# aniketntnu/WordDiffusion

Hardware: AMD Instinct MI355X
Metric: denoised 64x256 word images/sec (1000-step DDPM), whole job (higher is better)
Workload: dtype bf16x3; 1 GPU; BASELINE configs[1]: batch 64 per GPU of 64x256 crops = [64,4,8,32] latents, 1000-step DDPM (999 executed steps), base unet.py UNetModel (320 ch, mult (1,1), 4 heads, 339 writers), random-init synthetic weights; variant=base, batch_per_gpu=64, noise_steps=1000, executed_steps_per_image=999, precision=split-bf16 MFMA x3, fp32 accumulate (<=1e-4 of the fp32 reference), output_finite=True

## Files before the change

include/wdiff_hip.h:

```cpp
#ifndef WDIFF_HIP_H
#define WDIFF_HIP_H

#include <stdint.h>

#ifdef __cplusplus
extern "C" {
#endif

#define WD_OK 0
#define WD_EINVAL (-1)
#define WD_ELAUNCH (-2)
#define WD_ESTATE (-3)

#define WD_ACT_NONE 0
#define WD_ACT_SILU 1
#define WD_ACT_GEGLU 2

typedef uint16_t wd_bf16;

#define WD_MAX_KSPLIT 64

typedef struct wd_src {
    const wd_bf16* hi;
    const wd_bf16* lo;
// ... 173 lines not shown
                   const wd_bf16* mq_pl, const wd_bf16* mot_pl, void* stream);

int wd_emb_combine(const float* time, const float* label, const int64_t* y, int num_classes, int T, int B, int ted,
                   wd_bf16* out_hi, wd_bf16* out_lo, int out_ld, void* stream);
int wd_select_rows(const float* table, const int32_t* t_dev, int batch, int64_t row_floats, int chunk, float* out,
                   void* stream);

int wd_emb_combine_mix(const float* time, const float* label, const int32_t* pairs, const float* mix, int num_classes, int T, int B,
                       int ted, wd_bf16* out_hi, wd_bf16* out_lo, int out_ld, void* stream);
int wd_label_mix(const float* label, const int32_t* pairs, const float* mix, int num_classes, int B, int ted, float* out,
                 void* stream);

int wd_xattn_pair(const float* x, int ld, int batch, int hw, int c, float eps, int heads, int L, const float* gamma_a,
                  const float* beta_a, const wd_bf16* mq_pl_a, const wd_bf16* mot_pl_a, const float* bias_a, const float* gamma_b,
                  const float* beta_b, const wd_bf16* mq_pl_b, const wd_bf16* mot_pl_b, const float* bias_b, float* out, int out_ld,
                  const float* gamma2, const float* beta2, float eps2, wd_bf16* n_hi, wd_bf16* n_lo, int n_ld, void* stream);

int wd_embed_tokens(const void* ids, int ids_are_i64, int rows, int seq_len, const float* table, int vocab, int c,
                    const float* pe, wd_bf16* out_hi, wd_bf16* out_lo, int out_ld, void* stream);

int wd_im2col3x3(const float* x, int batch, int cin, int h, int w, wd_bf16* out_hi, wd_bf16* out_lo, int kpad,
                 void* stream);

int wd_nchw_to_tokens(const float* x, int batch, int c, int hw, float* out, int ld, void* stream);
int wd_tokens_to_nchw(const float* x, int ld, int batch, int c, int hw, float* out, void* stream);

int wd_ddpm_step(float* x, const float* eps, int batch, int n_per_sample, const float* ca, const float* cb,
                 const float* cs, const int32_t* t_dev, const float* noise, uint64_t seed, uint64_t sample_offset,
                 void* stream);

int wd_ddpm_step_cfg(float* x, const float* first, const float* second, float scale, float* eps_out, int batch, int n_per_sample,
                     const float* ca, const float* cb, const float* cs, const int32_t* t_dev, const float* noise, uint64_t seed,
                     uint64_t sample_offset, void* stream);

int wd_advance_timestep(int32_t* t_dev, int delta, int64_t* t64, int batch, void* stream);

int wd_ddim_step(float* x, const float* eps, const float* second, float scale, float* eps_out, int batch, int n_per_sample,
                 const float* c1, const float* c2, const float* c3, const float* c4, const float* c5, const int32_t* k_dev,
                 const int32_t* t_dev, const float* noise, uint64_t seed, uint64_t sample_offset, void* stream);

int wd_next_timestep(int32_t* k_dev, const int32_t* tau, int S, int32_t* t_dev, int64_t* t64, int batch, void* stream);

int wd_randn(float* out, int batch, int n_per_sample, uint64_t seed, uint64_t sample_offset, uint32_t stream_id,
             void* stream);

#define WD_VAE_MAX_LATENT 8
// ... 142 lines not shown
```

worddiffusion_amd/_native.py:

```python
from __future__ import annotations

import ctypes as C
import os
import re

_HERE = os.path.dirname(os.path.abspath(__file__))
LIB_PATH = os.environ.get("WDIFF_LIB") or os.path.join(_HERE, "libwdiff_hip.so")
HEADER_PATH = os.path.join(os.path.dirname(_HERE), "include", "wdiff_hip.h")

WD_OK, WD_EINVAL, WD_ELAUNCH, WD_ESTATE = 0, -1, -2, -3
ACT_NONE, ACT_SILU, ACT_GEGLU = 0, 1, 2
VAE_MAX_LATENT, STREAM_VAE_POSTERIOR = 8, 3
NCLASS = 13
CLASS_NAMES = ("gemm", "gn_stats", "gn_apply", "layernorm", "attention", "other", "gemm_other_tiles", "gemm_splitk_reduce",
               "gemm_two_per_cu", "gemm_weights_to_registers", "feed_forward_fused", "weight_gradient", "gemm_small_maps_whole_k")

_vp = C.c_void_p
_i = C.c_int
_f = C.c_float
_u64 = C.c_uint64


class WdSrc(C.Structure):
    _fields_ = [("hi", _vp), ("lo", _vp), ("gather", _vp), ("ld", C.c_int32), ("c", C.c_int32),
# ... 56 lines not shown
    "wd_gemm_pack_w": (_i, [_vp, _vp, _i, _i, _vp, _vp, _vp]),
    "wd_ff_fused": (_i, [C.POINTER(WdFfArgs), _vp]),
    "wd_ff_supported": (_i, [_i, _i]),
    "wd_ff_args_bytes": (_i, []),
    "wd_gemm_args_bytes": (_i, []),
    "wd_gemm_experimental": (_i, []),
    "wd_gn_nchunk": (_i, [_i]),
    "wd_gn_stats": (_i, [_vp, _i, _i, _i, _i, _i, _vp, _vp]),
    "wd_gn_fold_chunks": (_i, [_vp, _i, _i, _i, _vp, _vp]),
    "wd_gn_conv3x3_few_supported": (_i, [_i, _i, _i]),
    "wd_gn_conv3x3_few": (_i, [_vp, _i, _i, _i, _i, _i, _i, _vp, _i, _i, _vp, _vp, _f, _i, _vp, _vp, _i, _vp, _vp]),
    "wd_gn_apply": (_i, [_vp, _i, _i, _i, _i, _i, _vp, _i, _i, _vp, _vp, _f, _i, _vp, _vp, _i, _i, _vp, _vp, _vp]),
    "wd_gn_apply2": (_i, [_vp, _i, _i, _vp, _i, _i, _i, _vp, _i, _i, _vp, _i, _i, _i, _i, _i, _i, _vp, _vp, _f, _i, _vp, _vp, _i, _vp,
                          _vp, _vp, _vp]),
    "wd_layernorm": (_i, [_vp, _i, _i, _i, _vp, _vp, _f, _vp, _vp, _i, _vp]),
    "wd_split": (_i, [_vp, _i, _i, _i, _i, _vp, _vp, _i, _vp]),
    "wd_attention": (_i, [_vp, _i, _vp, _i, _vp, _i, _i, _i, _i, _i, _i, _f, _vp, _vp, _vp, _i, _i, _i, _vp]),
    "wd_attention_packed_elems": (C.c_int64, [_i, _i, _i, _i]),
    "wd_attention_pack_kv": (_i, [_vp, _i, _vp, _i, _i, _i, _i, _i, _vp, _vp]),
    "wd_attention_packed": (_i, [_vp, _i, _vp, _i, _i, _i, _i, _i, _f, _vp, _vp, _vp, _i, _i, _i, _vp]),
    "wd_timestep_embedding": (_i, [_vp, _i, _vp, _i, _vp, _vp, _i, _vp]),
    "wd_embed_tokens": (_i, [_vp, _i, _i, _i, _vp, _i, _i, _vp, _vp, _vp, _i, _vp]),
    "wd_im2col3x3": (_i, [_vp, _i, _i, _i, _i, _vp, _vp, _i, _vp]),
    "wd_nchw_to_tokens": (_i, [_vp, _i, _i, _i, _vp, _i, _vp]),
    "wd_tokens_to_nchw": (_i, [_vp, _i, _i, _i, _i, _vp, _vp]),
    "wd_ddpm_step": (_i, [_vp, _vp, _i, _i, _vp, _vp, _vp, _vp, _vp, _u64, _u64, _vp]),
    "wd_advance_timestep": (_i, [_vp, _i, _vp, _i, _vp]),
    "wd_randn": (_i, [_vp, _i, _i, _u64, _u64, C.c_uint32, _vp]),
    "wd_vae_posterior": (_i, [_vp, _i, _vp, _vp, _i, _i, _i, _vp, _vp, _vp, _f, _vp, _u64, _u64, _vp]),
    "wd_posterior_sample": (_i, [_vp, _vp, _i, _i, _vp, _f, _vp, _u64, _u64, _vp]),
    "wd_noise_images": (_i, [_vp, _vp, _vp, _vp, _vp, _i, _i, _vp, _vp]),
    "wd_copy2d": (_i, [_vp, C.c_int64, _vp, C.c_int64, C.c_int64, C.c_int64, _vp]),
    "wd_ema_update": (_i, [_vp, _vp, C.c_int64, C.c_double, _vp]),
    "wd_adamw_table_entry_bytes": (_i, []),
    "wd_adamw_chunk": (_i, []),
    "wd_adamw_multi": (_i, [_vp, _i, C.c_int64, C.c_double, C.c_double, C.c_double, C.c_double, C.c_double, C.c_int64, _i,
                           C.c_double, _vp]),
    "wd_mse_loss": (_i, [_vp, _vp, C.c_int64, _vp, _vp, _vp, _i, _vp]),
    "wd_transpose_planes": (_i, [_vp, _vp, _i, _i, _i, _vp, _i, _i, _i, _i, _i, _i, _vp, _vp, _vp]),
    "wd_repack_entry_bytes": (_i, []),
    "wd_repack_tile": (_i, []),
    "wd_repack_vchunk": (_i, []),
    "wd_repack_multi": (_i, [_vp, _i, C.c_int64, _vp]),
    "wd_attention_bwd_scratch_floats": (C.c_int64, [_i, _i, _i, _i]),
    "wd_attention_bwd": (_i, [_vp, _i, _vp, _i, _vp, _i, _vp, _i, _i, _i, _i, _i, _i, _f, _vp, _i, _vp, _i, _vp, _i, _vp, C.c_int64, _vp]),
    "wd_xattn_supported": (_i, [_i, _i, _i]),
# ... 95 lines not shown
```

worddiffusion_amd/build.py:

```python
from __future__ import annotations

import hashlib
import json
import os
import subprocess
import sys
from concurrent.futures import ThreadPoolExecutor

HERE = os.path.dirname(os.path.abspath(__file__))
CSRC = os.path.join(HERE, "csrc")
LIB = os.path.join(HERE, "libwdiff_hip.so")
SOURCES = ["wd_gemm.hip", "wd_gemmw.hip", "wd_gemmq.hip", "wd_ff.hip", "wd_dw.hip", "wd_norm.hip", "wd_attn.hip", "wd_xattn.hip", "wd_misc.hip", "wd_train.hip", "wd_bwd.hip", "wd_pack.hip", "wd_runtime.hip"]
HEADERS = [os.path.join(CSRC, "wd_common.h"), os.path.join(CSRC, "wd_gemm_epi.h"), os.path.join(CSRC, "wd_gemm_priv.h"), os.path.join(os.path.dirname(HERE), "include", "wdiff_hip.h")]
FLAGS = ["-O3", "--offload-arch=gfx950", "-fPIC", "-std=c++17", "-fno-gpu-rdc"]
FILE_FLAGS = {"wd_attn.hip": ["-mllvm", "-amdgpu-mfma-vgpr-form=1"]}
if os.environ.get("WDIFF_EXPERIMENTAL", "0") != "0":
    FLAGS.append("-DWDIFF_EXPERIMENTAL")
if os.environ.get("WDIFF_STAMPS", "0") != "0":
    FLAGS += ["-DWD_DW_STAMPS", "-DWD_GEMMW_STAMPS", "-DWD_Q_STAMPS"]


def _hipcc() -> str:
    for cand in (os.environ.get("HIPCC"), "/opt/rocm/bin/hipcc", "hipcc"):
        if cand and (os.path.isabs(cand) and os.path.exists(cand) or not os.path.isabs(cand)):
            return cand
    return "hipcc"


def _digest(paths) -> str:
    h = hashlib.sha256()
    for p in paths:
        with open(p, "rb") as f:
            h.update(hashlib.sha256(f.read()).digest())
    h.update(" ".join(FLAGS + FILE_FLAGS.get(os.path.basename(paths[0]), [])).encode())
    return h.hexdigest()
# ... 55 lines not shown
```

worddiffusion_amd/csrc/wd_norm.hip:

```cpp
#include "wd_common.h"

namespace {

constexpr int GN_TOK = 32;

__global__ void gn_stats_kernel(const float* __restrict__ x, int ld, int hw, int c, int cpg, int nchunk,
                                double* __restrict__ part) {
    extern __shared__ __attribute__((aligned(16))) char smem[];
    float* s_sum = reinterpret_cast<float*>(smem);
    float* s_sq = s_sum + 2 * c;
    const int b = blockIdx.y, j = blockIdx.x;
    const int cx = threadIdx.x * 4;
    const int t0 = j * GN_TOK, t1 = min(hw, t0 + GN_TOK);
    if (cx < c) {
        float4 s = make_float4(0, 0, 0, 0), q = make_float4(0, 0, 0, 0);
        const float* base = x + ((long)b * hw) * ld + cx;
        for (int t = t0 + threadIdx.y; t < t1; t += 2) {
            const float4 v = *reinterpret_cast<const float4*>(base + (long)t * ld);
            s.x += v.x; s.y += v.y; s.z += v.z; s.w += v.w;
            q.x += v.x * v.x; q.y += v.y * v.y; q.z += v.z * v.z; q.w += v.w * v.w;
        }
        *reinterpret_cast<float4*>(s_sum + threadIdx.y * c + cx) = s;
        *reinterpret_cast<float4*>(s_sq + threadIdx.y * c + cx) = q;
    }
// ... 166 lines not shown
    }
}

__global__ void split_kernel(const float* __restrict__ x, int ld, int rows, int c, int silu,
                             wd_bf16* __restrict__ out_hi, wd_bf16* __restrict__ out_lo, int out_ld) {
    const int c4 = c >> 2;
    const long total = (long)rows * c4;
    for (long i = (long)blockIdx.x * blockDim.x + threadIdx.x; i < total; i += (long)gridDim.x * blockDim.x) {
        const long r = i / c4;
        const int cx = (int)(i - r * c4) * 4;
        float4 v = *reinterpret_cast<const float4*>(x + r * ld + cx);
        if (silu) {
            v.x = wd_silu(v.x); v.y = wd_silu(v.y); v.z = wd_silu(v.z); v.w = wd_silu(v.w);
        }
        uint2 h, l;
        wd_split4(v, h, l);
        *reinterpret_cast<uint2*>(out_hi + r * out_ld + cx) = h;
        if (out_lo) *reinterpret_cast<uint2*>(out_lo + r * out_ld + cx) = l;
    }
}

constexpr int GC_CH = 64;
constexpr int GC_PITCH = GC_CH + 4;
template <int PXL>
__global__ void __launch_bounds__(256) gn_conv_few_kernel(const float* __restrict__ x, int ld, int H, int W, int c, int cpg, int nchunk,
                                                         int part_cpg, const double* __restrict__ part,
                                                         const float* __restrict__ gamma, const float* __restrict__ beta, float eps,
                                                         int silu, const float* __restrict__ w, const float* __restrict__ bias, int oc,
                                                         float* __restrict__ out) {
    constexpr int CG = 256 / PXL, CPT = GC_CH / CG;
    constexpr int NLD = 3 * PXL * (GC_CH / 4) / 256;
    extern __shared__ __attribute__((aligned(16))) char smem[];
    float* s_w = reinterpret_cast<float*>(smem);
    float* s_t = s_w + 9 * GC_CH * 4;
    __shared__ float s_mean[32], s_rstd[32];
    const int b = blockIdx.x, y = blockIdx.y, tid = threadIdx.x;
    const int hw = H * W, ng = c / cpg;
    float4 pv[NLD];
    auto request = [&](int c0) {
#pragma unroll
        for (int k = 0; k < NLD; ++k) {
            const int i = tid + 256 * k;
            const int r = i / (PXL * (GC_CH / 4)), rem = i - r * (PXL * (GC_CH / 4));
            const int px = rem / (GC_CH / 4), c4 = rem - px * (GC_CH / 4);
            const int yy = y + r - 1;
            pv[k] = (yy >= 0 && yy < H && px < W)
                        ? *reinterpret_cast<const float4*>(x + ((long)b * hw + (long)yy * W + px) * ld + c0 + c4 * 4)
                        : make_float4(0.f, 0.f, 0.f, 0.f);
        }
    };
    request(0);
    if (tid < ng) {
        const int ratio = cpg / part_cpg, ngs = c / part_cpg;
        double ds = 0.0, dq = 0.0;
        for (int j = 0; j < nchunk; ++j) {
            const double* p = part + (((long)b * nchunk + j) * ngs + tid * ratio) * 2;
            for (int k = 0; k < ratio; ++k) {
                ds += p[2 * k];
                dq += p[2 * k + 1];
            }
        }
        const double n = (double)hw * cpg;
        const double mean = ds / n;
        double var = dq / n - mean * mean;
        if (var < 0.0) var = 0.0;
        s_mean[tid] = (float)mean;
        s_rstd[tid] = (float)(1.0 / sqrt(var + (double)eps));
    }
    for (int i = tid; i < 3 * 2 * (GC_CH / 4); i += 256) {
        const int r = i / (2 * (GC_CH / 4)), rem = i - r * (2 * (GC_CH / 4));
        const int side = rem / (GC_CH / 4), c4 = rem - side * (GC_CH / 4);
        *reinterpret_cast<float4*>(s_t + ((long)r * (W + 2) + (side ? W + 1 : 0)) * GC_PITCH + c4 * 4) = make_float4(0.f, 0.f, 0.f, 0.f);
    }
    for (int i = tid; i < 9 * GC_CH; i += 256) *reinterpret_cast<float4*>(s_w + (long)i * 4) = make_float4(0.f, 0.f, 0.f, 0.f);
    __syncthreads();
    const int pl = tid % PXL, cg = tid / PXL;
    float4 acc = make_float4(0.f, 0.f, 0.f, 0.f);
    for (int c0 = 0; c0 < c; c0 += GC_CH) {
        for (int i = tid; i < oc * GC_CH * 9; i += 256) {
            const int o = i / (GC_CH * 9), rem = i - o * (GC_CH * 9);
            s_w[rem * 4 + o] = w[((long)o * c + c0) * 9 + rem];
        }
        float sc[4], sh[4];
        {
            const int ch = c0 + (tid & (GC_CH / 4 - 1)) * 4;
#pragma unroll
            for (int j = 0; j < 4; ++j) {
                const int g = (ch + j) / cpg;
                sc[j] = s_rstd[g] * gamma[ch + j];
                sh[j] = beta[ch + j] - s_mean[g] * sc[j];
            }
        }
#pragma unroll
        for (int k = 0; k < NLD; ++k) {
            const int i = tid + 256 * k;
            const int r = i / (PXL * (GC_CH / 4)), rem = i - r * (PXL * (GC_CH / 4));
            const int px = rem / (GC_CH / 4), c4 = rem - px * (GC_CH / 4);
            const int yy = y + r - 1;
            if (px >= W) continue;
            float4 o = make_float4(0.f, 0.f, 0.f, 0.f);
            if (yy >= 0 && yy < H) {
                const float4 v = pv[k];
                o = make_float4(v.x * sc[0] + sh[0], v.y * sc[1] + sh[1], v.z * sc[2] + sh[2], v.w * sc[3] + sh[3]);
                if (silu) {
                    o.x = wd_silu(o.x); o.y = wd_silu(o.y); o.z = wd_silu(o.z); o.w = wd_silu(o.w);
                }
            }
            *reinterpret_cast<float4*>(s_t + ((long)r * (W + 2) + px + 1) * GC_PITCH + c4 * 4) = o;
        }
        if (c0 + GC_CH < c) request(c0 + GC_CH);
        __syncthreads();
        if (pl < W) {
#pragma unroll
            for (int dy = 0; dy < 3; ++dy)
#pragma unroll
                for (int dx = 0; dx < 3; ++dx) {
                    const float* at = s_t + ((long)dy * (W + 2) + pl + dx) * GC_PITCH + cg * CPT;
                    const float* wt = s_w + ((long)(cg * CPT) * 9 + dy * 3 + dx) * 4;
#pragma unroll
                    for (int k = 0; k < CPT / 4; ++k) {
                        const float4 a = *reinterpret_cast<const float4*>(at + 4 * k);
                        const float4 w0 = *reinterpret_cast<const float4*>(wt + (4 * k + 0) * 36);
                        const float4 w1 = *reinterpret_cast<const float4*>(wt + (4 * k + 1) * 36);
                        const float4 w2 = *reinterpret_cast<const float4*>(wt + (4 * k + 2) * 36);
                        const float4 w3 = *reinterpret_cast<const float4*>(wt + (4 * k + 3) * 36);
                        acc.x += a.x * w0.x; acc.y += a.x * w0.y; acc.z += a.x * w0.z; acc.w += a.x * w0.w;
                        acc.x += a.y * w1.x; acc.y += a.y * w1.y; acc.z += a.y * w1.z; acc.w += a.y * w1.w;
                        acc.x += a.z * w2.x; acc.y += a.z * w2.y; acc.z += a.z * w2.z; acc.w += a.z * w2.w;
                        acc.x += a.w * w3.x; acc.y += a.w * w3.y; acc.z += a.w * w3.z; acc.w += a.w * w3.w;
                    }
                }
        }
        __syncthreads();
    }
    float* s_red = s_t;
    *reinterpret_cast<float4*>(s_red + ((long)cg * PXL + pl) * 4) = acc;
    __syncthreads();
    for (int i = tid; i < W * oc; i += 256) {
        const int o = i / W, px = i - o * W;
        float v = bias ? bias[o] : 0.f;
        for (int g = 0; g < CG; ++g) v += s_red[((long)g * PXL + px) * 4 + o];
        out[(((long)b * oc + o) * H + y) * W + px] = v;
    }
}

__global__ void __launch_bounds__(256) gn_fold_chunks_kernel(const double* __restrict__ part, int nchunk, int ng2,
                                                            double* __restrict__ out) {
    __shared__ double red[4][64];
    const int col = threadIdx.x & 63, lane = threadIdx.x >> 6;
    const long b = blockIdx.x;
    double acc = 0.0;
    if (col < ng2)
        for (int j = lane; j < nchunk; j += 4) acc += part[(b * nchunk + j) * ng2 + col];
    red[lane][col] = acc;
    __syncthreads();
    if (lane == 0 && col < ng2) out[b * ng2 + col] = (red[0][col] + red[1][col]) + (red[2][col] + red[3][col]);
}

}

extern "C" int wd_gn_nchunk(int hw) { return (hw + GN_TOK - 1) / GN_TOK; }

extern "C" int wd_gn_fold_chunks(const double* part, int batch, int nchunk, int ngroups, double* out, void* stream) {
    if (!part || !out || batch <= 0 || nchunk <= 0 || ngroups <= 0 || ngroups > 32) return WD_EINVAL;
    hipStream_t st = reinterpret_cast<hipStream_t>(stream);
// ... 27 lines not shown
                       silu, out_hi, out_lo, out_ld, raw_hi, raw_lo);
    return wd_check_launch();
}

extern "C" int wd_gn_apply2(const float* xa, int lda, int ca, const double* part_a, int nchunk_a, int part_cpg_a, int c_off_a,
                            const float* xb, int ldb, int cb, const double* part_b, int nchunk_b, int part_cpg_b, int c_off_b,
                            int batch, int hw, int cpg, const float* gamma, const float* beta, float eps, int silu,
                            wd_bf16* out_hi, wd_bf16* out_lo, int out_ld, wd_bf16* raw_hi, wd_bf16* raw_lo, const int32_t* perm_a,
                            void* stream) {
    if (!xa || !xb || !part_a || !part_b || !gamma || !beta || !out_hi || batch <= 0 || hw <= 0 || nchunk_a <= 0 || nchunk_b <= 0 ||
        part_cpg_a <= 0 || part_cpg_b <= 0)
        return WD_EINVAL;
    if (ca % 4 || cb % 4 || lda % 4 || ldb % 4 || out_ld % 4 || c_off_a % 4 || c_off_b % 4 || ca % cpg || cb % cpg ||
        ca / cpg > 32 || cb / cpg > 32 || cpg % part_cpg_a || cpg % part_cpg_b)
        return WD_EINVAL;
    hipStream_t st = reinterpret_cast<hipStream_t>(stream);
    WdLaunchScope scope(WD_CLS_GNAPPLY, st);
    const GnSrc s0 = {xa, part_a, lda, ca, nchunk_a, part_cpg_a, c_off_a, perm_a}, s1 = {xb, part_b, ldb, cb, nchunk_b, part_cpg_b, c_off_b, nullptr};
    hipLaunchKernelGGL(gn_apply_kernel, dim3((hw + AP_TOK - 1) / AP_TOK, batch, 2), dim3(256), 0, st, s0, s1, hw, cpg, gamma, beta, eps,
                       silu, out_hi, out_lo, out_ld, raw_hi, raw_lo);
    return wd_check_launch();
}

static int gn_conv_tile_floats(int w) { return 3 * (w + 2) * GC_PITCH > 1024 ? 3 * (w + 2) * GC_PITCH : 1024; }

extern "C" int wd_gn_conv3x3_few_supported(int c, int w, int oc) {
    return c > 0 && c % GC_CH == 0 && w > 0 && w <= 64 && oc >= 1 && oc <= 4 &&
           (size_t)(9 * GC_CH * 4 + gn_conv_tile_floats(w)) * sizeof(float) <= 64 * 1024;
}

extern "C" int wd_gn_conv3x3_few(const float* x, int ld, int batch, int h, int w, int c, int cpg, const double* part, int nchunk,
                                 int part_cpg, const float* gamma, const float* beta, float eps, int silu, const float* weight,
                                 const float* bias, int oc, float* out, void* stream) {
    if (!x || !part || !gamma || !beta || !weight || !out || batch <= 0 || h <= 0 || nchunk <= 0 || part_cpg <= 0) return WD_EINVAL;
    if (!wd_gn_conv3x3_few_supported(c, w, oc) || ld % 4 || cpg <= 0 || c % cpg || c / cpg > 32 || cpg % part_cpg) return WD_EINVAL;
    hipStream_t st = reinterpret_cast<hipStream_t>(stream);
    const size_t smem = (size_t)(9 * GC_CH * 4 + gn_conv_tile_floats(w)) * sizeof(float);
    WdLaunchScope scope(WD_CLS_OTHER, st);
    if (w <= 32)
        hipLaunchKernelGGL(gn_conv_few_kernel<32>, dim3(batch, h), dim3(256), smem, st, x, ld, h, w, c, cpg, nchunk, part_cpg, part,
                           gamma, beta, eps, silu, weight, bias, oc, out);
    else
        hipLaunchKernelGGL(gn_conv_few_kernel<64>, dim3(batch, h), dim3(256), smem, st, x, ld, h, w, c, cpg, nchunk, part_cpg, part,
                           gamma, beta, eps, silu, weight, bias, oc, out);
    return wd_check_launch();
}

extern "C" int wd_layernorm(const float* x, int ld, int rows, int c, const float* gamma, const float* beta, float eps,
                            wd_bf16* out_hi, wd_bf16* out_lo, int out_ld, void* stream) {
    if (!x || !gamma || !beta || !out_hi || rows <= 0 || c <= 0) return WD_EINVAL;
    if (c % 4 || ld % 4 || out_ld % 4 || c > 64 * 4 * LN_MAX4) return WD_EINVAL;
    hipStream_t st = reinterpret_cast<hipStream_t>(stream);
    WdLaunchScope scope(WD_CLS_LN, st);
    hipLaunchKernelGGL(layernorm_kernel, dim3((rows + 3) / 4), dim3(256), 0, st, x, ld, rows, c, gamma, beta, eps,
                       out_hi, out_lo, out_ld);
    return wd_check_launch();
}

extern "C" int wd_split(const float* x, int ld, int rows, int c, int silu, wd_bf16* out_hi, wd_bf16* out_lo, int out_ld,
                        void* stream) {
    if (!x || !out_hi || rows <= 0 || c <= 0 || c % 4 || ld % 4 || out_ld % 4) return WD_EINVAL;
    hipStream_t st = reinterpret_cast<hipStream_t>(stream);
    const long total = (long)rows * (c / 4);
    const int grid = (int)((total + 255) / 256 < 2048 ? (total + 255) / 256 : 2048);
    WdLaunchScope scope(WD_CLS_OTHER, st);
    hipLaunchKernelGGL(split_kernel, dim3(grid), dim3(256), 0, st, x, ld, rows, c, silu, out_hi, out_lo, out_ld);
    return wd_check_launch();
// ... 2 lines not shown
```

worddiffusion_amd/engine.py:

```python
from __future__ import annotations

import ctypes as C
import math
import os
from typing import Dict, List, Optional, Tuple

import numpy as np
import torch

from . import _native as N
from .layers import (DownsampleParams, ResBlockParams, SpatialTransformerParams, UpsampleParams)


def conv_gather_table(h: int, w: int, mode: str) -> Tuple[np.ndarray, int, int]:
    if mode == "same":
        ho, wo = h, w
    elif mode == "down":
        ho, wo = (h + 2 - 3) // 2 + 1, (w + 2 - 3) // 2 + 1
    elif mode == "up":
        ho, wo = 2 * h, 2 * w
    elif mode == "down_rb":
        ho, wo = (h - 2) // 2 + 1, (w - 2) // 2 + 1
    else:
        raise ValueError(mode)
# ... 274 lines not shown
        self._pack = None
        self._w: Dict[str, torch.Tensor] = {}
        self._w3: Dict[str, torch.Tensor] = {}
        self._w3_meta: Dict[str, tuple] = {}
        self._wf: Dict[str, torch.Tensor] = {}
        self.use_wdirect = os.environ.get("WDIFF_GEMM_WDIRECT", "1") != "0"
        self.use_up_phases = os.environ.get("WDIFF_UPSAMPLE_PHASES", "1") != "0"
        self._derived: Dict[str, tuple] = {}
        self.use_smallmap = os.environ.get("WDIFF_GEMM_SMALLMAP", "1") != "0"
        self.fuse_ff = os.environ.get("WDIFF_FUSE_FF", "1") != "0"
        self.fuse_proj = os.environ.get("WDIFF_FUSE_PROJ", "1") != "0"
        self.fuse_ln = os.environ.get("WDIFF_FUSE_LN", "1") != "0"
        self.fuse_gn_in = int(os.environ.get("WDIFF_FUSE_GN_IN", "1"))
        self.use_slab = os.environ.get("WDIFF_SLAB", "0") != "0"
        self.fuse_stats = os.environ.get("WDIFF_FUSE_STATS", "1") != "0"
        self.fuse_xattn = os.environ.get("WDIFF_FUSE_XATTN", "1") != "0"
        self.use_conv3 = os.environ.get("WDIFF_CONV3", "0") != "0"
        if (self.use_slab or self.use_conv3) and not self.lib.wd_gemm_experimental():
            raise N.NativeError("WDIFF_SLAB / WDIFF_CONV3 need a library built with WDIFF_EXPERIMENTAL=1 "
                                "(python -m worddiffusion_amd.build --force)")
        self.fuse_xattn_pair = os.environ.get("WDIFF_FUSE_XATTN_PAIR", "1") != "0"
        self.fuse_st = os.environ.get("WDIFF_FUSE_ST", "1") != "0"
        self.fuse_out = os.environ.get("WDIFF_FUSE_OUT", "1") != "0"
        self.pack_kv = os.environ.get("WDIFF_PACK_KV", "1") != "0"
        self.fuse_gn2 = os.environ.get("WDIFF_FUSE_GN2", "1") != "0"
        self.fuse_gn = os.environ.get("WDIFF_FUSE_GN", "1") != "0"
        self.fuse_split = os.environ.get("WDIFF_FUSE_SPLIT", "1") != "0"
        self._plans: Dict[tuple, Plan] = {}
        self._tabs: Dict[tuple, torch.Tensor] = {}
        self._tab_np: Dict[int, np.ndarray] = {}
        self._same_w: Dict[int, int] = {}
        self._down_w: Dict[int, int] = {}
        self._ws = None
        self.device = None

    def set_precision(self, mode: str):
        npass = {"bf16x3": 3, "fp32": 3, "bf16": 1}[mode]
        if npass != self.npass:
            self.npass = npass
            self._plans.clear()

    def _recipes(self) -> "RecipeBook":
        m = self.model
        R = RecipeBook()
        film_w = []
        self.film_off = {}
        off = 0
        cin_conv = m.input_blocks[0][0]
        self.kpad_in = ((9 * cin_conv.in_channels + 31) // 32) * 32
        R.matrix("in.w", cin_conv.out_channels, self.kpad_in).fwd(cin_conv.weight)
        R.vector("in.b", cin_conv.bias)
        R.linear("te0", m.time_embed[0])
        R.linear("te2", m.time_embed[2])
        if m.num_classes is not None:
            R.vector("label", m.label_emb.weight)
        we = m.word_emb
        cd = we.embedding.weight.shape[1]
        R.vector("we.table", we.embedding.weight)
        qkv = (we.attention.linear_query, we.attention.linear_key, we.attention.linear_value)
        R.matrix("we.qkv.w", 3 * cd, cd)
        R.vector_cat("we.qkv.b", [l.bias for l in qkv])
        for i, l in enumerate(qkv):
            R["we.qkv.w"].fwd(l.weight, row_off=i * cd)
        kv_w = []
        self.kv_off = {}
        kvo = 0
        for name, mod in self._walk():
            if isinstance(mod, ResBlockParams):
                R.vector(name + ".gn1.g", mod.in_layers[0].weight)
                R.vector(name + ".gn1.b", mod.in_layers[0].bias)
                R.matrix(name + ".c1.w", mod.cout, 9 * mod.cin).fwd(mod.in_layers[2].weight)
                R.vector(name + ".c1.b", mod.in_layers[2].bias)
                R.vector(name + ".gn2.g", mod.out_layers[0].weight)
                R.vector(name + ".gn2.b", mod.out_layers[0].bias)
# ... 883 lines not shown
                                                self._film.data_ptr()), "film rows of step t, second forward")
        else:
            if mix:
                P.pairs = torch.zeros((B, 2), dtype=torch.int32, device=dev)
                lab_rows = self._f32(P, B, ted)
                id_rows = torch.arange(B, dtype=torch.int64, device=dev)
                P.keep.append(id_rows)
                step.append((lib.wd_label_mix, (self._w["label"].data_ptr(), P.pairs.data_ptr(), P.mix_m.data_ptr(), m.num_classes,
                                                B, ted, lab_rows.data_ptr()), "blended label rows"))
            te = self._planes(P, B, mc)
            step.append((lib.wd_timestep_embedding, (P.t_in.data_ptr(), B, self._w["freqs"].data_ptr(), mc // 2,
                                                     te[0].data_ptr(), te[1].data_ptr() if lo_ok else None, mc),
                         "timestep_embedding"))
            e1 = self._planes(P, B, ted)
            self._gemm(step, "time_embed.0", [self._src(te, mc)], "te0.w", B, 1, bias=self._w["te0.b"], act=N.ACT_SILU,
                       out_pl=e1)
            e2 = self._planes(P, B, ted)
            self._gemm(step, "time_embed.2+label", [self._src(e1, ted)], "te2.w", B, 1, bias=self._w["te2.b"],
                       resid=(lab_rows if mix else self._w["label"]).data_ptr() if has_lab else None, resid_ld=ted if has_lab else 0,
                       resid_rows=(id_rows if mix else P.y_in).data_ptr() if has_lab else None, act=N.ACT_SILU, out_pl=e2)
            self._gemm(step, "emb_layers(all)", [self._src(e2, ted)], "film.w", B, 1, bias=self._w["film.b"],
                       out_f32=self._film, out_ld=self.film_total)

        xin = self._planes(P, B * H * W, self.kpad_in)
        step.append((lib.wd_im2col3x3, (P.x_in.data_ptr(), B, m.in_channels, H, W, xin[0].data_ptr(),
                                        xin[1].data_ptr() if lo_ok else None, self.kpad_in), "im2col"))
        h0 = self._f32(P, B * H * W, mc)
        g0 = self._gemm(step, "input_blocks.0", [self._src(xin, self.kpad_in)], "in.w", B * H * W, H * W,
                        bias=self._w["in.b"], out_f32=h0, out_ld=mc, want_stats=True)
        cur = Act(h0, mc, H, W, g0._stats)
        hs = [cur]

        def run_layers(prefix, blk, cur, extra=None):
            for j, mod in enumerate(blk):
                name = f"{prefix}.{j}"
                if isinstance(mod, ResBlockParams):
                    cur = self._resblock(P, name, mod, [cur] + ([extra] if (extra is not None and j == 0) else []))
                elif isinstance(mod, SpatialTransformerParams):
                    cur = self._transformer(P, name, mod, cur)
                elif isinstance(mod, DownsampleParams):
                    cur = self._resample(P, name, mod, cur, "down")
                elif isinstance(mod, UpsampleParams):
                    cur = self._resample(P, name, mod, cur, "up")
                else:
                    raise TypeError(type(mod))
            return cur

        for i, blk in enumerate(m.input_blocks):
            if i == 0:
                continue
            cur = run_layers(f"in{i}", blk, cur)
            hs.append(cur)
        cur = run_layers("mid", m.middle_block, cur)
# ... 105 lines not shown
```

Measured before the change: 34.36 images/s.

## Add direct fp32 input conv kernel and retile GN+conv3x3 output kernel

Replaces the im2col plus split-bf16 GEMM for the 4-channel input convolution with a direct fp32 kernel. It reads NCHW, keeps weights in registers, writes token-major output, and emits GroupNorm partial statistics. It also rewrites the GN-fused few-output conv3x3 kernel to use 4x16 spatial tiles, 512 threads, double-buffered weight and activation prefetch, and DPP lane shifts for horizontal neighbours. The aim is to remove the im2col round trip and launch, and to raise parallelism in the output conv. The cost is large register use (36 float4 weights per thread), and the accumulation order changes numerics slightly.

```diff
diff --git a/include/wdiff_hip.h b/include/wdiff_hip.h
--- a/include/wdiff_hip.h
+++ b/include/wdiff_hip.h
@@ -219,6 +219,11 @@
 int wd_im2col3x3(const float* x, int batch, int cin, int h, int w, wd_bf16* out_hi, wd_bf16* out_lo, int kpad,
                  void* stream);
 
+int wd_conv3x3_in_supported(int cin, int h, int w, int cout);
+int wd_conv3x3_in_nchunk(int hw);
+int wd_conv3x3_in(const float* x, int batch, int cin, int h, int w, const float* weight, const float* bias, int cout, float* out,
+                  int ld, double* part, int stat_cpg, void* stream);
+
 int wd_nchw_to_tokens(const float* x, int batch, int c, int hw, float* out, int ld, void* stream);
 int wd_tokens_to_nchw(const float* x, int ld, int batch, int c, int hw, float* out, void* stream);
 
diff --git a/worddiffusion_amd/_native.py b/worddiffusion_amd/_native.py
--- a/worddiffusion_amd/_native.py
+++ b/worddiffusion_amd/_native.py
@@ -102,6 +102,9 @@
     "wd_timestep_embedding": (_i, [_vp, _i, _vp, _i, _vp, _vp, _i, _vp]),
     "wd_embed_tokens": (_i, [_vp, _i, _i, _i, _vp, _i, _i, _vp, _vp, _vp, _i, _vp]),
     "wd_im2col3x3": (_i, [_vp, _i, _i, _i, _i, _vp, _vp, _i, _vp]),
+    "wd_conv3x3_in_supported": (_i, [_i, _i, _i, _i]),
+    "wd_conv3x3_in_nchunk": (_i, [_i]),
+    "wd_conv3x3_in": (_i, [_vp, _i, _i, _i, _i, _vp, _vp, _i, _vp, _i, _vp, _i, _vp]),
     "wd_nchw_to_tokens": (_i, [_vp, _i, _i, _i, _vp, _i, _vp]),
     "wd_tokens_to_nchw": (_i, [_vp, _i, _i, _i, _i, _vp, _vp]),
     "wd_ddpm_step": (_i, [_vp, _vp, _i, _i, _vp, _vp, _vp, _vp, _vp, _u64, _u64, _vp]),
diff --git a/worddiffusion_amd/build.py b/worddiffusion_amd/build.py
--- a/worddiffusion_amd/build.py
+++ b/worddiffusion_amd/build.py
@@ -10,7 +10,7 @@
 HERE = os.path.dirname(os.path.abspath(__file__))
 CSRC = os.path.join(HERE, "csrc")
 LIB = os.path.join(HERE, "libwdiff_hip.so")
-SOURCES = ["wd_gemm.hip", "wd_gemmw.hip", "wd_gemmq.hip", "wd_ff.hip", "wd_dw.hip", "wd_norm.hip", "wd_attn.hip", "wd_xattn.hip", "wd_misc.hip", "wd_train.hip", "wd_bwd.hip", "wd_pack.hip", "wd_runtime.hip"]
+SOURCES = ["wd_gemm.hip", "wd_gemmw.hip", "wd_gemmq.hip", "wd_ff.hip", "wd_dw.hip", "wd_norm.hip", "wd_attn.hip", "wd_xattn.hip", "wd_misc.hip", "wd_conv_in.hip", "wd_train.hip", "wd_bwd.hip", "wd_pack.hip", "wd_runtime.hip"]
 HEADERS = [os.path.join(CSRC, "wd_common.h"), os.path.join(CSRC, "wd_gemm_epi.h"), os.path.join(CSRC, "wd_gemm_priv.h"), os.path.join(os.path.dirname(HERE), "include", "wdiff_hip.h")]
 FLAGS = ["-O3", "--offload-arch=gfx950", "-fPIC", "-std=c++17", "-fno-gpu-rdc"]
 FILE_FLAGS = {"wd_attn.hip": ["-mllvm", "-amdgpu-mfma-vgpr-form=1"]}
diff --git a/worddiffusion_amd/csrc/wd_conv_in.hip b/worddiffusion_amd/csrc/wd_conv_in.hip
--- /dev/null
+++ b/worddiffusion_amd/csrc/wd_conv_in.hip
@@ -0,0 +1,147 @@
+#include "wd_common.h"
+
+namespace {
+
+constexpr int CI_NT = 512;
+constexpr int CI_TOK = 64;
+constexpr int CI_MAX_PIX = 2048;
+constexpr int CI_WBATCH = 12;
+constexpr int CI_WPAD = 4;
+
+__host__ __device__ inline size_t ci_scratch_bytes(int cin, int cout, bool stats) {
+    const size_t wb = (size_t)cin * 9 * (cout + CI_WPAD) * sizeof(float);
+    const size_t sb = stats ? ((size_t)(CI_NT / (cout / 4)) * cout + cout) * 2 * sizeof(double) : 0;
+    return wb > sb ? wb : sb;
+}
+
+template <int CIN>
+__global__ void __launch_bounds__(CI_NT) conv3x3_in_kernel(const float* __restrict__ x, int H, int W, const float* __restrict__ w,
+                                                          const float* __restrict__ bias, int cout, float* __restrict__ out, int ld,
+                                                          double* __restrict__ part, int cpg) {
+    constexpr int K = CIN * 9;
+    extern __shared__ __attribute__((aligned(16))) char smem[];
+    float4* s_x = reinterpret_cast<float4*>(smem);
+    float* s_w = reinterpret_cast<float*>(s_x + (H + 2) * (W + 2));
+    double* s_st = reinterpret_cast<double*>(s_w);
+    const int chunk = blockIdx.x, b = blockIdx.y, tid = threadIdx.x;
+    const int hw = H * W, pw = W + 2, wp = cout + CI_WPAD;
+    for (int i = tid; i < (H + 2) * pw; i += CI_NT) {
+        const int yy = i / pw - 1, xx = i % pw - 1;
+        float v[4] = {0.f, 0.f, 0.f, 0.f};
+        if (yy >= 0 && yy < H && xx >= 0 && xx < W) {
+#pragma unroll
+            for (int ci = 0; ci < CIN; ++ci) v[ci] = x[(((long)b * CIN + ci) * H + yy) * W + xx];
+        }
+        s_x[i] = make_float4(v[0], v[1], v[2], v[3]);
+    }
+    for (int i0 = 0; i0 < cout * K; i0 += CI_NT * CI_WBATCH) {
+        float v[CI_WBATCH];
+#pragma unroll
+        for (int u = 0; u < CI_WBATCH; ++u) v[u] = w[min(i0 + u * CI_NT + tid, cout * K - 1)];
+#pragma unroll
+        for (int u = 0; u < CI_WBATCH; ++u) {
+            const int i = i0 + u * CI_NT + tid, co = i / K, k = i - co * K;
+            if (i < cout * K) s_w[k * wp + co] = v[u];
+        }
+    }
+    const int nq = cout >> 2, ntl = CI_NT / nq;
+    const int tl = tid / nq, q = tid - tl * nq;
+    const bool active = tl < ntl;
+    __syncthreads();
+    float4 wr[K], bs = make_float4(0.f, 0.f, 0.f, 0.f);
+    if (active) {
+#pragma unroll
+        for (int k = 0; k < K; ++k) wr[k] = *reinterpret_cast<const float4*>(s_w + k * wp + 4 * q);
+        if (bias) bs = make_float4(bias[4 * q], bias[4 * q + 1], bias[4 * q + 2], bias[4 * q + 3]);
+    }
+    const int t0 = chunk * CI_TOK, nt = min(CI_TOK, hw - t0);
+    double su[4] = {0.0, 0.0, 0.0, 0.0}, sq[4] = {0.0, 0.0, 0.0, 0.0};
+    if (active) {
+        for (int t = tl; t < nt; t += ntl) {
+            const int p = t0 + t, y = p / W, xx = p - y * W;
+            const float4* px = s_x + y * pw + xx;
+            float acc[4] = {bs.x, bs.y, bs.z, bs.w};
+#pragma unroll
+            for (int tap = 0; tap < 9; ++tap) {
+                const float4 a4 = px[(tap / 3) * pw + tap % 3];
+                const float a[4] = {a4.x, a4.y, a4.z, a4.w};
+#pragma unroll
+                for (int ci = 0; ci < CIN; ++ci) {
+                    const float4 w4 = wr[ci * 9 + tap];
+                    acc[0] += w4.x * a[ci]; acc[1] += w4.y * a[ci]; acc[2] += w4.z * a[ci]; acc[3] += w4.w * a[ci];
+                }
+            }
+            *reinterpret_cast<float4*>(out + ((long)b * hw + p) * ld + 4 * q) = make_float4(acc[0], acc[1], acc[2], acc[3]);
+            if (part) {
+#pragma unroll
+                for (int o = 0; o < 4; ++o) {
+                    const double d = (double)acc[o];
+                    su[o] += d;
+                    sq[o] += d * d;
+                }
+            }
+        }
+    }
+    if (!part) return;
+    __syncthreads();
+    if (active) {
+#pragma unroll
+        for (int o = 0; o < 4; ++o) {
+            s_st[((long)tl * cout + 4 * q + o) * 2] = su[o];
+            s_st[((long)tl * cout + 4 * q + o) * 2 + 1] = sq[o];
+        }
+    }
+    __syncthreads();
+    double* s_ch = s_st + (long)ntl * cout * 2;
+    for (int ch = tid; ch < cout; ch += CI_NT) {
+        double ds = 0.0, dq = 0.0;
+        for (int l = 0; l < ntl; ++l) {
+            ds += s_st[((long)l * cout + ch) * 2];
+            dq += s_st[((long)l * cout + ch) * 2 + 1];
+        }
+        s_ch[2 * ch] = ds;
+        s_ch[2 * ch + 1] = dq;
+    }
+    __syncthreads();
+    const int ng = cout / cpg;
+    for (int g = tid; g < ng; g += CI_NT) {
+        double ds = 0.0, dq = 0.0;
+        for (int k = 0; k < cpg; ++k) {
+            ds += s_ch[2 * (g * cpg + k)];
+            dq += s_ch[2 * (g * cpg + k) + 1];
+        }
+        double* o = part + (((long)b * gridDim.x + chunk) * ng + g) * 2;
+        o[0] = ds;
+        o[1] = dq;
+    }
+}
+
+}
+
+extern "C" int wd_conv3x3_in_nchunk(int hw) { return (hw + CI_TOK - 1) / CI_TOK; }
+
+extern "C" int wd_conv3x3_in_supported(int cin, int h, int w, int cout) {
+    return cin >= 1 && cin <= 4 && h > 0 && w > 0 && w <= 64 && (long)(h + 2) * (w + 2) <= CI_MAX_PIX && cout >= 4 && cout % 4 == 0 &&
+           cout / 4 <= CI_NT && (size_t)(h + 2) * (w + 2) * sizeof(float4) + ci_scratch_bytes(cin, cout, true) <= 64 * 1024;
+}
+
+extern "C" int wd_conv3x3_in(const float* x, int batch, int cin, int h, int w, const float* weight, const float* bias, int cout,
+                             float* out, int ld, double* part, int stat_cpg, void* stream) {
+    if (!x || !weight || !out || batch <= 0 || batch > 65535 || !wd_conv3x3_in_supported(cin, h, w, cout)) return WD_EINVAL;
+    if (ld < cout || ld % 4) return WD_EINVAL;
+    if (part && (stat_cpg <= 0 || cout % stat_cpg)) return WD_EINVAL;
+    hipStream_t st = reinterpret_cast<hipStream_t>(stream);
+    const size_t smem = (size_t)(h + 2) * (w + 2) * sizeof(float4) + ci_scratch_bytes(cin, cout, part != nullptr);
+    const dim3 grid(wd_conv3x3_in_nchunk(h * w), batch);
+    WdLaunchScope scope(WD_CLS_OTHER, st, 2.0 * batch * h * w * (double)cout * 9 * cin);
+#define WD_CI_LAUNCH(CIN) \
+    hipLaunchKernelGGL(conv3x3_in_kernel<CIN>, grid, dim3(CI_NT), smem, st, x, h, w, weight, bias, cout, out, ld, part, stat_cpg)
+    switch (cin) {
+        case 1: WD_CI_LAUNCH(1); break;
+        case 2: WD_CI_LAUNCH(2); break;
+        case 3: WD_CI_LAUNCH(3); break;
+        default: WD_CI_LAUNCH(4); break;
+    }
+#undef WD_CI_LAUNCH
+    return wd_check_launch();
+}
diff --git a/worddiffusion_amd/csrc/wd_norm.hip b/worddiffusion_amd/csrc/wd_norm.hip
--- a/worddiffusion_amd/csrc/wd_norm.hip
+++ b/worddiffusion_amd/csrc/wd_norm.hip
@@ -212,125 +212,178 @@
 
 constexpr int GC_CH = 64;
 constexpr int GC_PITCH = GC_CH + 4;
-template <int PXL>
-__global__ void __launch_bounds__(256) gn_conv_few_kernel(const float* __restrict__ x, int ld, int H, int W, int c, int cpg, int nchunk,
-                                                         int part_cpg, const double* __restrict__ part,
-                                                         const float* __restrict__ gamma, const float* __restrict__ beta, float eps,
-                                                         int silu, const float* __restrict__ w, const float* __restrict__ bias, int oc,
-                                                         float* __restrict__ out) {
-    constexpr int CG = 256 / PXL, CPT = GC_CH / CG;
-    constexpr int NLD = 3 * PXL * (GC_CH / 4) / 256;
-    extern __shared__ __attribute__((aligned(16))) char smem[];
-    float* s_w = reinterpret_cast<float*>(smem);
-    float* s_t = s_w + 9 * GC_CH * 4;
+constexpr int GC_TR = 4, GC_TC = 16;
+constexpr int GC_NT = 512, GC_SLOTS = GC_NT / GC_TC, GC_CPS = GC_CH / GC_SLOTS;
+constexpr int GC_ITEMS = (GC_TR + 2) * (GC_TC + 2) * (GC_CH / 4);
+constexpr int GC_NLD = (GC_ITEMS + GC_NT - 1) / GC_NT;
+constexpr int GC_NWV = (4 * GC_CH * 9 + GC_NT - 1) / GC_NT;
+constexpr int GC_TILE_FLOATS = (GC_TR + 2) * (GC_TC + 2) * GC_PITCH;
+constexpr int GC_RED_FLOATS = GC_SLOTS * GC_TR * GC_TC * 4;
+static_assert(GC_CPS == 2, "a lane reads its two channels of a pixel as one float2");
+
+__device__ __forceinline__ float gc_from_left(float old, float v) {
+    return __int_as_float(__builtin_amdgcn_update_dpp(__float_as_int(old), __float_as_int(v), 0x111, 0xf, 0xf, false));
+}
+__device__ __forceinline__ float gc_from_right(float old, float v) {
+    return __int_as_float(__builtin_amdgcn_update_dpp(__float_as_int(old), __float_as_int(v), 0x101, 0xf, 0xf, false));
+}
+
+__global__ void __launch_bounds__(GC_NT) gn_conv_few_kernel(const float* __restrict__ x, int ld, int H, int W, int c, int cpg, int nchunk,
+                                                           int part_cpg, const double* __restrict__ part,
+                                                           const float* __restrict__ gamma, const float* __restrict__ beta, float eps,
+                                                           int silu, const float* __restrict__ w, const float* __restrict__ bias, int oc,
+                                                           float* __restrict__ out) {
+    __shared__ __attribute__((aligned(16))) float s_t[GC_TILE_FLOATS > GC_RED_FLOATS ? GC_TILE_FLOATS : GC_RED_FLOATS];
+    __shared__ __attribute__((aligned(16))) float s_w[GC_CH * 9 * 4];
     __shared__ float s_mean[32], s_rstd[32];
-    const int b = blockIdx.x, y = blockIdx.y, tid = threadIdx.x;
+    const int b = blockIdx.x, x0 = blockIdx.y * GC_TC, y0 = blockIdx.z * GC_TR, tid = threadIdx.x;
     const int hw = H * W, ng = c / cpg;
-    float4 pv[NLD];
-    auto request = [&](int c0) {
-#pragma unroll
-        for (int k = 0; k < NLD; ++k) {
-            const int i = tid + 256 * k;
-            const int r = i / (PXL * (GC_CH / 4)), rem = i - r * (PXL * (GC_CH / 4));
+    struct Pre {
+        float4 pv[GC_NLD], ga, be;
+        float wv[GC_NWV];
+    };
+    const int cq = (tid & (GC_CH / 4 - 1)) * 4;
+    auto request = [&](Pre& P, int c0w) {
+        const int c0 = min(c0w, c - GC_CH);
+#pragma unroll
+        for (int k = 0; k < GC_NLD; ++k) {
+            const int i = tid + GC_NT * k;
+            const int r = i / ((GC_TC + 2) * (GC_CH / 4)), rem = i - r * ((GC_TC + 2) * (GC_CH / 4));
             const int px = rem / (GC_CH / 4), c4 = rem - px * (GC_CH / 4);
-            const int yy = y + r - 1;
-            pv[k] = (yy >= 0 && yy < H && px < W)
-                        ? *reinterpret_cast<const float4*>(x + ((long)b * hw + (long)yy * W + px) * ld + c0 + c4 * 4)
-                        : make_float4(0.f, 0.f, 0.f, 0.f);
-        }
+            const int yy = min(max(y0 + r - 1, 0), H - 1), xx = min(max(x0 + px - 1, 0), W - 1);
+            P.pv[k] = *reinterpret_cast<const float4*>(x + ((long)b * hw + (long)yy * W + xx) * ld + c0 + c4 * 4);
+        }
+#pragma unroll
+        for (int k = 0; k < GC_NWV; ++k) {
+            const int i = min(tid + GC_NT * k, 4 * GC_CH * 9 - 1);
+            const int o = i / (GC_CH * 9), rem = i - o * (GC_CH * 9);
+            P.wv[k] = w[((long)min(o, oc - 1) * c + c0) * 9 + rem];
+        }
+        P.ga = make_float4(gamma[c0 + cq], gamma[c0 + cq + 1], gamma[c0 + cq + 2], gamma[c0 + cq + 3]);
+        P.be = make_float4(beta[c0 + cq], beta[c0 + cq + 1], beta[c0 + cq + 2], beta[c0 + cq + 3]);
     };
-    request(0);
-    if (tid < ng) {
-        const int ratio = cpg / part_cpg, ngs = c / part_cpg;
-        double ds = 0.0, dq = 0.0;
-        for (int j = 0; j < nchunk; ++j) {
-            const double* p = part + (((long)b * nchunk + j) * ngs + tid * ratio) * 2;
-            for (int k = 0; k < ratio; ++k) {
-                ds += p[2 * k];
-                dq += p[2 * k + 1];
-            }
-        }
-        const double n = (double)hw * cpg;
-        const double mean = ds / n;
-        double var = dq / n - mean * mean;
-        if (var < 0.0) var = 0.0;
-        s_mean[tid] = (float)mean;
-        s_rstd[tid] = (float)(1.0 / sqrt(var + (double)eps));
-    }
-    for (int i = tid; i < 3 * 2 * (GC_CH / 4); i += 256) {
-        const int r = i / (2 * (GC_CH / 4)), rem = i - r * (2 * (GC_CH / 4));
-        const int side = rem / (GC_CH / 4), c4 = rem - side * (GC_CH / 4);
-        *reinterpret_cast<float4*>(s_t + ((long)r * (W + 2) + (side ? W + 1 : 0)) * GC_PITCH + c4 * 4) = make_float4(0.f, 0.f, 0.f, 0.f);
-    }
-    for (int i = tid; i < 9 * GC_CH; i += 256) *reinterpret_cast<float4*>(s_w + (long)i * 4) = make_float4(0.f, 0.f, 0.f, 0.f);
+    Pre pa, pb;
+    request(pa, 0);
+    request(pb, GC_CH);
+    {
+        double* s_ps = reinterpret_cast<double*>(s_t);
+        const int g = tid & 31, jl = tid >> 5;
+        if (g < ng) {
+            const int ratio = cpg / part_cpg, ngs = c / part_cpg;
+            double ds = 0.0, dq = 0.0;
+            for (int j = jl; j < nchunk; j += GC_NT / 32) {
+                const double* p = part + (((long)b * nchunk + j) * ngs + g * ratio) * 2;
+                for (int k = 0; k < ratio; ++k) {
+                    ds += p[2 * k];
+                    dq += p[2 * k + 1];
+                }
+            }
+            s_ps[(jl * 32 + g) * 2] = ds;
+            s_ps[(jl * 32 + g) * 2 + 1] = dq;
+        }
+        __syncthreads();
+        if (tid < ng) {
+            double ds = 0.0, dq = 0.0;
+            for (int l = 0; l < GC_NT / 32; ++l) {
+                ds += s_ps[(l * 32 + tid) * 2];
+                dq += s_ps[(l * 32 + tid) * 2 + 1];
+            }
+            const double n = (double)hw * cpg;
+            const double mean = ds / n;
+            double var = dq / n - mean * mean;
+            if (var < 0.0) var = 0.0;
+            s_mean[tid] = (float)mean;
+            s_rstd[tid] = (float)(1.0 / sqrt(var + (double)eps));
+        }
+    }
     __syncthreads();
-    const int pl = tid % PXL, cg = tid / PXL;
-    float4 acc = make_float4(0.f, 0.f, 0.f, 0.f);
-    for (int c0 = 0; c0 < c; c0 += GC_CH) {
-        for (int i = tid; i < oc * GC_CH * 9; i += 256) {
+    const int lx = tid & (GC_TC - 1), slot = tid / GC_TC;
+    const bool edge = lx == 0 || lx == GC_TC - 1;
+    const float* at = s_t + (lx + 1) * GC_PITCH + slot * GC_CPS;
+    const float* ah = s_t + (lx == 0 ? 0 : GC_TC + 1) * GC_PITCH + slot * GC_CPS;
+    const float* wt = s_w + slot * GC_CPS * 36;
+    float acc[GC_TR][4];
+#pragma unroll
+    for (int r = 0; r < GC_TR; ++r)
+#pragma unroll
+        for (int o = 0; o < 4; ++o) acc[r][o] = 0.f;
+    auto chunk = [&](Pre& P, int c0) {
+#pragma unroll
+        for (int k = 0; k < GC_NWV; ++k) {
+            const int i = tid + GC_NT * k;
             const int o = i / (GC_CH * 9), rem = i - o * (GC_CH * 9);
-            s_w[rem * 4 + o] = w[((long)o * c + c0) * 9 + rem];
+            if (o < 4) s_w[rem * 4 + o] = o < oc ? P.wv[k] : 0.f;
         }
         float sc[4], sh[4];
         {
-            const int ch = c0 + (tid & (GC_CH / 4 - 1)) * 4;
+            const float ga[4] = {P.ga.x, P.ga.y, P.ga.z, P.ga.w}, be[4] = {P.be.x, P.be.y, P.be.z, P.be.w};
 #pragma unroll
             for (int j = 0; j < 4; ++j) {
-                const int g = (ch + j) / cpg;
-                sc[j] = s_rstd[g] * gamma[ch + j];
-                sh[j] = beta[ch + j] - s_mean[g] * sc[j];
-            }
-        }
-#pragma unroll
-        for (int k = 0; k < NLD; ++k) {
-            const int i = tid + 256 * k;
-            const int r = i / (PXL * (GC_CH / 4)), rem = i - r * (PXL * (GC_CH / 4));
+                const int g = (c0 + cq + j) / cpg;
+                sc[j] = s_rstd[g] * ga[j];
+                sh[j] = be[j] - s_mean[g] * sc[j];
+            }
+        }
+#pragma unroll
+        for (int k = 0; k < GC_NLD; ++k) {
+            const int i = tid + GC_NT * k;
+            if (i >= GC_ITEMS) continue;
+            const int r = i / ((GC_TC + 2) * (GC_CH / 4)), rem = i - r * ((GC_TC + 2) * (GC_CH / 4));
             const int px = rem / (GC_CH / 4), c4 = rem - px * (GC_CH / 4);
-            const int yy = y + r - 1;
-            if (px >= W) continue;
+            const int yy = y0 + r - 1, xx = x0 + px - 1;
             float4 o = make_float4(0.f, 0.f, 0.f, 0.f);
-            if (yy >= 0 && yy < H) {
-                const float4 v = pv[k];
+            if (yy >= 0 && yy < H && xx >= 0 && xx < W) {
+                const float4 v = P.pv[k];
                 o = make_float4(v.x * sc[0] + sh[0], v.y * sc[1] + sh[1], v.z * sc[2] + sh[2], v.w * sc[3] + sh[3]);
                 if (silu) {
                     o.x = wd_silu(o.x); o.y = wd_silu(o.y); o.z = wd_silu(o.z); o.w = wd_silu(o.w);
                 }
             }
-            *reinterpret_cast<float4*>(s_t + ((long)r * (W + 2) + px + 1) * GC_PITCH + c4 * 4) = o;
-        }
-        if (c0 + GC_CH < c) request(c0 + GC_CH);
+            *reinterpret_cast<float4*>(s_t + (r * (GC_TC + 2) + px) * GC_PITCH + c4 * 4) = o;
+        }
+        request(P, c0 + 2 * GC_CH);
         __syncthreads();
-        if (pl < W) {
-#pragma unroll
-            for (int dy = 0; dy < 3; ++dy)
-#pragma unroll
-                for (int dx = 0; dx < 3; ++dx) {
-                    const float* at = s_t + ((long)dy * (W + 2) + pl + dx) * GC_PITCH + cg * CPT;
-                    const float* wt = s_w + ((long)(cg * CPT) * 9 + dy * 3 + dx) * 4;
-#pragma unroll
-                    for (int k = 0; k < CPT / 4; ++k) {
-                        const float4 a = *reinterpret_cast<const float4*>(at + 4 * k);
-                        const float4 w0 = *reinterpret_cast<const float4*>(wt + (4 * k + 0) * 36);
-                        const float4 w1 = *reinterpret_cast<const float4*>(wt + (4 * k + 1) * 36);
-                        const float4 w2 = *reinterpret_cast<const float4*>(wt + (4 * k + 2) * 36);
-                        const float4 w3 = *reinterpret_cast<const float4*>(wt + (4 * k + 3) * 36);
-                        acc.x += a.x * w0.x; acc.y += a.x * w0.y; acc.z += a.x * w0.z; acc.w += a.x * w0.w;
-                        acc.x += a.y * w1.x; acc.y += a.y * w1.y; acc.z += a.y * w1.z; acc.w += a.y * w1.w;
-                        acc.x += a.z * w2.x; acc.y += a.z * w2.y; acc.z += a.z * w2.z; acc.w += a.z * w2.w;
-                        acc.x += a.w * w3.x; acc.y += a.w * w3.y; acc.z += a.w * w3.z; acc.w += a.w * w3.w;
-                    }
+        float a[GC_TR + 2][3][GC_CPS];
+#pragma unroll
+        for (int r = 0; r < GC_TR + 2; ++r) {
+            const float2 ce = *reinterpret_cast<const float2*>(at + r * (GC_TC + 2) * GC_PITCH);
+            float2 ha = make_float2(0.f, 0.f);
+            if (edge) ha = *reinterpret_cast<const float2*>(ah + r * (GC_TC + 2) * GC_PITCH);
+            a[r][1][0] = ce.x; a[r][1][1] = ce.y;
+            a[r][0][0] = gc_from_left(ha.x, ce.x); a[r][0][1] = gc_from_left(ha.y, ce.y);
+            a[r][2][0] = gc_from_right(ha.x, ce.x); a[r][2][1] = gc_from_right(ha.y, ce.y);
+        }
+#pragma unroll
+        for (int j = 0; j < GC_CPS; ++j)
+#pragma unroll
+            for (int t = 0; t < 9; ++t) {
+                const float4 w4 = *reinterpret_cast<const float4*>(wt + (j * 9 + t) * 4);
+#pragma unroll
+                for (int r = 0; r < GC_TR; ++r) {
+                    const float v = a[r + t / 3][t % 3][j];
+                    acc[r][0] += v * w4.x; acc[r][1] += v * w4.y; acc[r][2] += v * w4.z; acc[r][3] += v * w4.w;
                 }
-        }
+            }
         __syncthreads();
+    };
+    for (int c0 = 0;; c0 += 2 * GC_CH) {
+        chunk(pa, c0);
+        if (c0 + GC_CH >= c) break;
+        chunk(pb, c0 + GC_CH);
+        if (c0 + 2 * GC_CH >= c) break;
     }
     float* s_red = s_t;
-    *reinterpret_cast<float4*>(s_red + ((long)cg * PXL + pl) * 4) = acc;
+#pragma unroll
+    for (int r = 0; r < GC_TR; ++r)
+        *reinterpret_cast<float4*>(s_red + ((slot * GC_TR + r) * GC_TC + lx) * 4) = make_float4(acc[r][0], acc[r][1], acc[r][2], acc[r][3]);
     __syncthreads();
-    for (int i = tid; i < W * oc; i += 256) {
-        const int o = i / W, px = i - o * W;
+    for (int i = tid; i < GC_TR * GC_TC * oc; i += GC_NT) {
+        const int o = i / (GC_TR * GC_TC), p = i - o * (GC_TR * GC_TC);
+        const int yy = y0 + p / GC_TC, xx = x0 + p % GC_TC;
+        if (yy >= H || xx >= W) continue;
         float v = bias ? bias[o] : 0.f;
-        for (int g = 0; g < CG; ++g) v += s_red[((long)g * PXL + px) * 4 + o];
-        out[(((long)b * oc + o) * H + y) * W + px] = v;
+        for (int g = 0; g < GC_SLOTS; ++g) v += s_red[(g * GC_TR * GC_TC + p) * 4 + o];
+        out[(((long)b * oc + o) * H + yy) * W + xx] = v;
     }
 }
 
@@ -404,11 +457,8 @@
     return wd_check_launch();
 }
 
-static int gn_conv_tile_floats(int w) { return 3 * (w + 2) * GC_PITCH > 1024 ? 3 * (w + 2) * GC_PITCH : 1024; }
-
 extern "C" int wd_gn_conv3x3_few_supported(int c, int w, int oc) {
-    return c > 0 && c % GC_CH == 0 && w > 0 && w <= 64 && oc >= 1 && oc <= 4 &&
-           (size_t)(9 * GC_CH * 4 + gn_conv_tile_floats(w)) * sizeof(float) <= 64 * 1024;
+    return c > 0 && c % GC_CH == 0 && w > 0 && w <= 64 && oc >= 1 && oc <= 4;
 }
 
 extern "C" int wd_gn_conv3x3_few(const float* x, int ld, int batch, int h, int w, int c, int cpg, const double* part, int nchunk,
@@ -416,15 +466,11 @@
                                  const float* bias, int oc, float* out, void* stream) {
     if (!x || !part || !gamma || !beta || !weight || !out || batch <= 0 || h <= 0 || nchunk <= 0 || part_cpg <= 0) return WD_EINVAL;
     if (!wd_gn_conv3x3_few_supported(c, w, oc) || ld % 4 || cpg <= 0 || c % cpg || c / cpg > 32 || cpg % part_cpg) return WD_EINVAL;
-    hipStream_t st = reinterpret_cast<hipStream_t>(stream);
-    const size_t smem = (size_t)(9 * GC_CH * 4 + gn_conv_tile_floats(w)) * sizeof(float);
+    if ((h + GC_TR - 1) / GC_TR > 65535) return WD_EINVAL;
+    hipStream_t st = reinterpret_cast<hipStream_t>(stream);
     WdLaunchScope scope(WD_CLS_OTHER, st);
-    if (w <= 32)
-        hipLaunchKernelGGL(gn_conv_few_kernel<32>, dim3(batch, h), dim3(256), smem, st, x, ld, h, w, c, cpg, nchunk, part_cpg, part,
-                           gamma, beta, eps, silu, weight, bias, oc, out);
-    else
-        hipLaunchKernelGGL(gn_conv_few_kernel<64>, dim3(batch, h), dim3(256), smem, st, x, ld, h, w, c, cpg, nchunk, part_cpg, part,
-                           gamma, beta, eps, silu, weight, bias, oc, out);
+    hipLaunchKernelGGL(gn_conv_few_kernel, dim3(batch, (w + GC_TC - 1) / GC_TC, (h + GC_TR - 1) / GC_TR), dim3(GC_NT), 0, st, x, ld, h,
+                       w, c, cpg, nchunk, part_cpg, part, gamma, beta, eps, silu, weight, bias, oc, out);
     return wd_check_launch();
 }
 
diff --git a/worddiffusion_amd/engine.py b/worddiffusion_amd/engine.py
--- a/worddiffusion_amd/engine.py
+++ b/worddiffusion_amd/engine.py
@@ -320,6 +320,7 @@
         self.fuse_xattn_pair = os.environ.get("WDIFF_FUSE_XATTN_PAIR", "1") != "0"
         self.fuse_st = os.environ.get("WDIFF_FUSE_ST", "1") != "0"
         self.fuse_out = os.environ.get("WDIFF_FUSE_OUT", "1") != "0"
+        self.fuse_in = os.environ.get("WDIFF_FUSE_IN", "1") != "0"
         self.pack_kv = os.environ.get("WDIFF_PACK_KV", "1") != "0"
         self.fuse_gn2 = os.environ.get("WDIFF_FUSE_GN2", "1") != "0"
         self.fuse_gn = os.environ.get("WDIFF_FUSE_GN", "1") != "0"
@@ -348,6 +349,7 @@
         self.kpad_in = ((9 * cin_conv.in_channels + 31) // 32) * 32
         R.matrix("in.w", cin_conv.out_channels, self.kpad_in).fwd(cin_conv.weight)
         R.vector("in.b", cin_conv.bias)
+        R.vector("in.w.f32", cin_conv.weight)
         R.linear("te0", m.time_embed[0])
         R.linear("te2", m.time_embed[2])
         if m.num_classes is not None:
@@ -1277,13 +1279,25 @@
             self._gemm(step, "emb_layers(all)", [self._src(e2, ted)], "film.w", B, 1, bias=self._w["film.b"],
                        out_f32=self._film, out_ld=self.film_total)
 
-        xin = self._planes(P, B * H * W, self.kpad_in)
-        step.append((lib.wd_im2col3x3, (P.x_in.data_ptr(), B, m.in_channels, H, W, xin[0].data_ptr(),
-                                        xin[1].data_ptr() if lo_ok else None, self.kpad_in), "im2col"))
         h0 = self._f32(P, B * H * W, mc)
-        g0 = self._gemm(step, "input_blocks.0", [self._src(xin, self.kpad_in)], "in.w", B * H * W, H * W,
-                        bias=self._w["in.b"], out_f32=h0, out_ld=mc, want_stats=True)
-        cur = Act(h0, mc, H, W, g0._stats)
+        if self.fuse_in and self.variant != "phosc" and lib.wd_conv3x3_in_supported(m.in_channels, H, W, mc) and mc % 32 == 0:
+            stats = None
+            if self.fuse_stats:
+                nchunk = lib.wd_conv3x3_in_nchunk(H * W)
+                part = torch.zeros((B, nchunk, 32, 2), dtype=torch.float64, device=dev)
+                P.keep.append(part)
+                stats = (part, nchunk, mc // 32)
+            step.append((lib.wd_conv3x3_in, (P.x_in.data_ptr(), B, m.in_channels, H, W, self._w["in.w.f32"].data_ptr(),
+                                             self._w["in.b"].data_ptr(), mc, h0.data_ptr(), mc,
+                                             stats[0].data_ptr() if stats else None, mc // 32), "input_blocks.0: conv3x3 from NCHW"))
+            cur = Act(h0, mc, H, W, stats)
+        else:
+            xin = self._planes(P, B * H * W, self.kpad_in)
+            step.append((lib.wd_im2col3x3, (P.x_in.data_ptr(), B, m.in_channels, H, W, xin[0].data_ptr(),
+                                            xin[1].data_ptr() if lo_ok else None, self.kpad_in), "im2col"))
+            g0 = self._gemm(step, "input_blocks.0", [self._src(xin, self.kpad_in)], "in.w", B * H * W, H * W,
+                            bias=self._w["in.b"], out_f32=h0, out_ld=mc, want_stats=True)
+            cur = Act(h0, mc, H, W, g0._stats)
         hs = [cur]
 
         def run_layers(prefix, blk, cur, extra=None):
```

New measurement: 34.76 images/s (median of 6 runs). 1.2% higher.
